# phylo42/RAPPAS

Hardware: AMD Instinct MI355X
Metric: reads placed/sec (whole node), 150 bp DNA vs 10^7-kmer DB (higher is better)
Workload: dtype f32; 1 GPU; C2: DNA k=10, 999 branches, phylo-kmer DB of 786432 keys / 9995042 entries (seed 42), replicated per GPU; 10000000 x 150 symbol reads per GPU per step (uniform, seed 1+rank), keep_at_most=7; reads_per_gpu=10000000

## Files before the change

### rappas_amd/csrc/rk_kernels.hip

```cpp
#include "rk_device.h"
#include "rk_slots24.h"
#include "rk_compact32.h"
#include "rk_translate.h"
#include "rk_masses.h"
#include "rk_samples.h"

#include <type_traits>
#ifndef RK_ROW_NT
#define RK_ROW_NT 0
#endif
#ifndef RK_ROW_AUX
#define RK_ROW_AUX 0
#endif
#ifndef RK_HEADS_MAX_K
#define RK_HEADS_MAX_K 16
#endif
#ifndef RK_ABLATE
#define RK_ABLATE 0
#endif
#include "../../include/rappas_place.h"

namespace rk {

#ifdef RK_STAMPS
__device__ unsigned long long rk_stamp_buf[2 * 4096 * 16];
__device__ __forceinline__ unsigned long long rk_now() {
    unsigned long long t;
    __builtin_amdgcn_sched_barrier(0);
    asm volatile("s_memtime %0\n\ts_waitcnt lgkmcnt(0)" : "=s"(t)::"memory");
    __builtin_amdgcn_sched_barrier(0);
    return t;
}
struct Stamps {
    unsigned long long st_[16] = {0, 0, 0, 0, 0, 0, 0, 0, 0, 0, 0, 0, 0, 0, 0, 0};
    unsigned long long t_ = rk_now();
    __device__ __forceinline__ void mark(int slot) {
        const unsigned long long n_ = rk_now();
        st_[slot] += n_ - t_;
        t_ = n_;
    }
    __device__ __forceinline__ void add(int slot, unsigned long long n) { st_[slot] += n; }
    __device__ __forceinline__ void store(unsigned long long index) const {
        for (int i = 0; i < 16; i++) rk_stamp_buf[index * 16 + i] = st_[i];
    }
};
#else
struct Stamps {
    __device__ __forceinline__ void mark(int) {}
    __device__ __forceinline__ void add(int, unsigned long long) {}
    __device__ __forceinline__ void store(unsigned long long) const {}
};
#endif

__device__ __forceinline__ u32 ord_f32(float f) {
    u32 u = __float_as_uint(f);
    return (u & 0x80000000u) ? ~u : (u | 0x80000000u);
}
__device__ __forceinline__ float unord_f32(u32 o) {
    u32 u = (o & 0x80000000u) ? (o & 0x7FFFFFFFu) : ~o;
    return __uint_as_float(u);
}
__device__ __forceinline__ u64 make_key(u32 raw_score_bits, u32 branch) {
    return ((u64)ord_f32(__uint_as_float(raw_score_bits)) << 32) | (u64)(0xFFFFu - branch);
}
__device__ __forceinline__ u64 shfl64(u64 v, int src, int width) {
    u32 lo = (u32)v, hi = (u32)(v >> 32);
    lo = __shfl(lo, src, width);
    hi = __shfl(hi, src, width);
    return ((u64)hi << 32) | lo;
}
__device__ __forceinline__ u64 shfl_xor64(u64 v, int m, int width) {
    u32 lo = (u32)v, hi = (u32)(v >> 32);
    lo = __shfl_xor(lo, m, width);
    hi = __shfl_xor(hi, m, width);
    return ((u64)hi << 32) | lo;
}
__device__ __forceinline__ double shfl_f64(double v, int src, int width) {
    return __longlong_as_double((long long)shfl64((u64)__double_as_longlong(v), src, width));
}
__device__ __forceinline__ bool tile_order_given(const PlaceArgs &a) { return a.perm != nullptr && *a.keep_order == 0u; }
__device__ __forceinline__ u32 batch_class(const PlaceArgs &a) { return a.keep_order[0] == 0u ? 2u : (a.keep_order[3] != 0u ? 1u : 0u); }
__device__ __forceinline__ bool batch_is_mine(const PlaceArgs &a) {
    if (!a.only_if || !a.perm) return true;
    return ((a.only_if >> batch_class(a)) & 1u) != 0u;
}
__device__ __forceinline__ bool takes_only_marked(const PlaceArgs &a) {
    if (!a.only_marked) return false;
    if (!a.marked_if || !a.perm) return true;
    return ((a.marked_if >> batch_class(a)) & 1u) != 0u;
}
__device__ __forceinline__ u64 tile_read(const PlaceArgs &a, u64 slot, bool given) { return given ? (u64)a.perm[slot] : slot; }
struct ReadHead {
    u32 R, flags, Q;
    float QT;
    bool is_amb, rejected;
};
template <int BITS>
__device__ __forceinline__ void clamp_len(u32 &R, u32 words_per_read) {
    const u32 cap_syms = (words_per_read * 32u) / BITS;
    R = R < cap_syms ? R : cap_syms;
}
template <int BITS>
__device__ __forceinline__ ReadHead read_head(const PlaceArgs &a, u32 R_raw, u32 fin, bool have) {
    const u32 k = a.db.k;
    ReadHead h;
    h.R = R_raw;
    clamp_len<BITS>(h.R, a.words_per_read);
    h.flags = fin & (RK_FLAG_BAD_CHAR | RK_FLAG_AMBIGUOUS | RK_FLAG_TOO_LONG);
    h.is_amb = (fin & RK_FLAG_AMBIGUOUS) != 0;
    h.rejected = (fin & (RK_FLAG_BAD_CHAR | RK_FLAG_TOO_LONG)) != 0;
    if (h.R < k) h.flags |= RK_FLAG_TOO_SHORT;
    h.Q = (have && !h.is_amb && !h.rejected && h.R >= k) ? (h.R - k + 1) : 0u;
    h.QT = (float)(int)h.Q * a.db.T;
    return h;
}
__device__ __forceinline__ bool deferred(const PlaceArgs &a, const ReadHead &h) { return h.is_amb && a.has_ascii && !h.rejected; }
__device__ __forceinline__ void wave_lds_fence() {
    __builtin_amdgcn_fence(__ATOMIC_ACQ_REL, "wavefront");
    __builtin_amdgcn_wave_barrier();
}

template <int G>
__device__ __forceinline__ u64 group_bits(u64 bal, u32 gi) {
    if (G == 64) return bal;
    u32 lo = (u32)bal, hi = (u32)(bal >> 32);
    asm("" : "+v"(lo), "+v"(hi));
    if (G == 32) return gi ? hi : lo;
    constexpr u32 PER = 32 / (G < 32 ? G : 32);
    const u32 half = gi >= PER ? hi : lo;
    return (half >> ((gi % PER) * (u32)G)) & ((1u << (G < 32 ? G : 31)) - 1u);
}
template <int G>
__device__ __forceinline__ int count_below(u64 m, u32 li) {
    if (G <= 32) return __builtin_popcount((u32)m & ((1u << li) - 1u));
    return (int)__builtin_amdgcn_mbcnt_hi((u32)(m >> 32), __builtin_amdgcn_mbcnt_lo((u32)m, 0u));
}
__device__ __forceinline__ u64 bits_below(u32 n) {
    u32 lo = n >= 32u ? 0xFFFFFFFFu : ((1u << (n & 31u)) - 1u);
    u32 hi = n <= 32u ? 0u : (n >= 64u ? 0xFFFFFFFFu : ((1u << ((n - 32u) & 31u)) - 1u));
    asm("" : "+v"(lo), "+v"(hi));
    return ((u64)hi << 32) | lo;
}
__device__ __forceinline__ u64 place_bits(u32 v, u32 sh) {
    u32 lo = sh < 32u ? v << (sh & 31u) : 0u;
    u32 hi = sh >= 32u ? v << ((sh - 32u) & 31u) : ((sh & 31u) ? v >> ((32u - sh) & 31u) : 0u);
    asm("" : "+v"(lo), "+v"(hi));
    return ((u64)hi << 32) | lo;
}
__device__ __forceinline__ bool lane_bit(u64 m, u32 lane) {
    u32 lo = (u32)m, hi = (u32)(m >> 32);
    asm("" : "+v"(lo), "+v"(hi));
    return (((lane & 32u) ? hi : lo) >> (lane & 31u)) & 1u;
}
__device__ __forceinline__ u64 funnel96(u32 w0, u32 w1, u32 w2, u32 sh) {
    return ((u64)__builtin_amdgcn_alignbit(w2, w1, sh) << 32) | __builtin_amdgcn_alignbit(w1, w0, sh);
}

__device__ __forceinline__ void load_entry(const DbView &db, u64 desc, u32 e, u32 &br, float &sc) {
    const unsigned char *base = db.rows + ((desc >> DESC_LEN_BITS) << 3);
    if (db.soa) {
        const u32 len = (u32)desc & DESC_LEN_MASK;
        br = ((const unsigned short *)base)[e];
        sc = ((const float *)(base + 2 * (size_t)len))[e];
    } else {
        const Entry en = ((const Entry *)base)[e];
        br = en.branch ? (en.branch >> 2) - 1u : 0xFFFFu;
        sc = en.score;
    }
}

template <int BITS>
__device__ __forceinline__ u64 extract_code(const u32 *rec, u32 words, u32 j, u32 k) {
    const u32 bit = j * BITS;
    const u32 wi = bit >> 5, sh = bit & 31;
    const u32 last = words - 1;
    const u32 w0 = rec[wi];
    const u32 i1 = wi + 1 < words ? wi + 1 : last;
    u32 w1 = rec[i1];
    w1 = wi + 1 < words ? w1 : 0u;
    const u32 nbits = k * BITS;
    u32 w2 = 0u;
    if (BITS == 5 || nbits + 31 > 64) {
        const u32 i2 = wi + 2 < words ? wi + 2 : last;
        w2 = rec[i2];
        w2 = (wi + 2 < words && nbits + sh > 64) ? w2 : 0u;
    }
    const u64 code = funnel96(w0, w1, w2, sh);
    return nbits >= 64 ? code : (code & ((1ull << nbits) - 1));
}

template <int BITS>
__device__ __forceinline__ u64 dense_index(u64 code, u32 k) {
    if (BITS == 2) return code;
    if (k <= 7) {
        const u32 lo = (u32)code;
        u32 idx = (u32)(code >> 30) & 31u;
        idx = idx * 20u + ((lo >> 25) & 31u);
        idx = idx * 20u + ((lo >> 20) & 31u);
        idx = idx * 20u + ((lo >> 15) & 31u);
        idx = idx * 20u + ((lo >> 10) & 31u);
        idx = idx * 20u + ((lo >> 5) & 31u);
        idx = idx * 20u + (lo & 31u);
// ... 176 lines not shown
            const u32 xw = b - s_lo;
            return (xw < s_win) ? (xw + 1u) * 4u : 0u;
        }
        const u32 t = b - wlo4p4;
        return win ? ((t < w4) ? t + 4u : 0u) : b;
    };
    while (true) {
#pragma unroll
        for (int u = 0; u < U; u++) {
            apply_slot(S, slot_of(br[u]), sc[u], QT, T);
            cursor_issue<G, WIDE, SOA>(c, list, cnt, li, (int)li, rows, br[u], sc[u], s_lo, s_win);
        }
        if (!__any(c.h < cnt)) break;
    }
#pragma unroll
    for (int u = 0; u < U; u++) apply_slot(S, slot_of(br[u]), sc[u], QT, T);
}

template <bool WIDE> struct ItemT { typedef u32 type; };
template <> struct ItemT<true> { typedef u64 type; };

template <int G, bool WIDE>
__device__ __forceinline__ typename ItemT<WIDE>::type make_item(u64 off8, u32 n) {
    if (WIDE) return (typename ItemT<WIDE>::type)((off8 << DESC_LEN_BITS) | n);
    return (typename ItemT<WIDE>::type)((u32)(off8 >> 3) << 4 | (n >> 3));
}

template <int G, bool WIDE>
__device__ __forceinline__ void chunk_issue(typename ItemT<WIDE>::type it, bool in, u32 li, u32 li8,
                                            const unsigned char *rows, u32 &br, float &sc) {
    typedef typename OffsetT<WIDE>::type off_t;
    bool ok;
    off_t eo;
    if (WIDE) {
        const u32 n = (u32)it & DESC_LEN_MASK;
        ok = in && li < n;
        eo = (off_t)(((u64)it >> DESC_LEN_BITS) << 3) + li8;
    } else {
        ok = in && (li >> 3) < ((u32)it & 15u);
        eo = (off_t)((((u32)it & ~15u) << 2) + li8);
    }
    eo = ok ? eo : (off_t)0;
    if (RK_ABLATE & 16) eo = 0;
    const uint2 e = *(const uint2 *)(rows + eo);
    br = e.x;
    sc = __uint_as_float(e.y);
}

template <int G, int U, bool WIDE>
__device__ __forceinline__ void accumulate_chunks(u32 *S, u32 nb, const typename ItemT<WIDE>::type *items, int cnt,
                                                  u32 li, const unsigned char *rows, float QT, float T) {
    typedef typename ItemT<WIDE>::type item_t;
    const u32 li8 = li * 8;
    u32 br[U];
    float sc[U];
    item_t it[U];
#pragma unroll
    for (int u = 0; u < U; u++) chunk_issue<G, WIDE>(items[u], u < cnt, li, li8, rows, br[u], sc[u]);
#pragma unroll
    for (int u = 0; u < U; u++) it[u] = items[U + u];
    int s0 = 0;
    while (true) {
#pragma unroll
        for (int u = 0; u < U; u++) {
            apply_slot(S, br[u], sc[u], QT, T);
            chunk_issue<G, WIDE>(it[u], s0 + U + u < cnt, li, li8, rows, br[u], sc[u]);
            it[u] = items[s0 + 2 * U + u];
        }
        s0 += U;
        if (!__any(s0 < cnt)) break;
    }
}

constexpr u32 ITEM_FILLER = 0xFFFFFF00u;
typedef u32 v2u32 __attribute__((ext_vector_type(2)));

__device__ __forceinline__ __amdgpu_buffer_rsrc_t rows_resource(const DbView &db) {
    return __builtin_amdgcn_make_buffer_rsrc((void *)db.rows, (short)0, (int)(u32)db.rows_bytes, 0x00020000);
}

template <int G, int U, bool MONO, bool WIN = false, bool D24 = false>
__device__ __forceinline__ void accumulate_units(u32 *S, const u32 *items, int wcnt, u32 li,
                                                 __amdgpu_buffer_rsrc_t rs, float QT, float T, u32 wlo4p4 = 4u, u32 w4 = 0xFFFFFFFFu) {
    static_assert(!D24 || (G == 16 && !WIN), "dense units: 16-lane groups, whole trees");
    static_assert(rk_slots24::SLOT_BITS == SLOT24_BITS, "rk_slots24.h unpacks the slot words rk_device.h defines");
    const u32 li8 = li * 8;
    const u32 my_unit = li >> 4;
    const rk_slots24::Shifts sh24 = rk_slots24::lane_shifts(li);
    u32 sb[U], it[U];
    float sc[U];
    auto issue = [&](u32 item, u32 &b, float &v) {
        u32 off = item + li8;
        if (G > 16) off = (my_unit <= (item & 7u)) ? (item & ~127u) + li8 : ITEM_FILLER;
        if (RK_ABLATE & 16) off = li8;
        const v2u32 e = __builtin_amdgcn_raw_buffer_load_b64(rs, (int)off, 0, RK_ROW_AUX);
        b = e.x;
        v = __uint_as_float(e.y);
    };
    auto slot_of = [&](u32 b) {
        if (!WIN) return b;
        const u32 t = b - wlo4p4;
        return (t < w4) ? t + 4u : 0u;
    };
    auto prepare = [&](float v, u32 *&pa, u32 *&pb) {
        const int w = (int)__float_as_uint(v);
        const u32 r = (u32)__builtin_amdgcn_update_dpp(w, w, 0x128, 0xF, 0x3, false);
        const rk_slots24::Slots s = rk_slots24::lane_slots(sh24, r);
        pa = S + s.a;
        pb = S + s.b;
    };
#pragma unroll
    for (int u = 0; u < U; u++) issue(items[u], sb[u], sc[u]);
#pragma unroll
    for (int u = 0; u < U; u++) it[u] = items[U + u];
    int s0 = 0;
    if (D24) {
        u32 *pa, *pb;
        prepare(sc[0], pa, pb);
        while (true) {
#pragma unroll
            for (int u = 0; u < U; u++) {
                u32 *na, *nb;
                if (RK_ABLATE & 8) {
                    asm volatile("" ::"v"(pa), "v"(pb), "v"(sb[u]), "v"(sc[u]));
                    prepare(sc[(u + 1) % U], na, nb);
                } else {
                    const u32 oa = *pa, ob = *pb;
                    prepare(sc[(u + 1) % U], na, nb);
                    *pa = __float_as_uint(touch_base<MONO>(oa, QT) + __uint_as_float(sb[u]));
                    *pb = __float_as_uint(touch_base<MONO>(ob, QT) + sc[u]);
                }
                issue(it[u], sb[u], sc[u]);
                it[u] = items[s0 + 2 * U + u];
                pa = na;
                pb = nb;
            }
            s0 += U;
            if (s0 >= wcnt) break;
        }
        return;
    }
    while (true) {
#pragma unroll
        for (int u = 0; u < U; u++) {
            apply_slot<MONO>(S, slot_of(sb[u]), sc[u], QT, T);
            issue(it[u], sb[u], sc[u]);
            it[u] = items[s0 + 2 * U + u];
        }
        s0 += U;
        if (s0 >= wcnt) break;
    }
}

template <int S>
__device__ __forceinline__ u32 row_ror32(u32 v) {
    return (u32)__builtin_amdgcn_update_dpp(0, (int)v, 0x120 + S, 0xF, 0xF, false);
}
template <int G, int S>
__device__ __forceinline__ u64 group_rotate(u64 v, u32 li) {
    if (G == 16) {
        return ((u64)row_ror32<S>((u32)(v >> 32)) << 32) | row_ror32<S>((u32)v);
    } else {
        return shfl64(v, (int)((li + G - S) % G), G);
    }
}
template <int G, int S>
struct RankAbove {
    static __device__ __forceinline__ int run(u64 v, u32 li) {
        return ((group_rotate<G, S>(v, li) > v) ? 1 : 0) + RankAbove<G, S - 1>::run(v, li);
    }
};
template <int G>
struct RankAbove<G, 0> {
    static __device__ __forceinline__ int run(u64, u32) { return 0; }
};
template <int G>
__device__ __forceinline__ u64 group_max(u64 v) {
    if (G == 16) {
        u64 o;
        o = ((u64)row_ror32<8>((u32)(v >> 32)) << 32) | row_ror32<8>((u32)v); v = o > v ? o : v;
        o = ((u64)row_ror32<4>((u32)(v >> 32)) << 32) | row_ror32<4>((u32)v); v = o > v ? o : v;
        o = ((u64)row_ror32<2>((u32)(v >> 32)) << 32) | row_ror32<2>((u32)v); v = o > v ? o : v;
        o = ((u64)row_ror32<1>((u32)(v >> 32)) << 32) | row_ror32<1>((u32)v); v = o > v ? o : v;
        return v;
    } else {
#pragma unroll
        for (int s = 1; s < G; s <<= 1) {
            u64 o = shfl_xor64(v, s, G);
            v = o > v ? o : v;
        }
        return v;
    }
}

template <int G>
__device__ __forceinline__ int rank_candidates(const u64 *list, int c, u64 *win, int K, u32 li) {
    if (c <= G) {
        const u64 mine = ((int)li < c) ? list[li] : 0ull;
        const int rank = RankAbove<G, G - 1>::run(mine, li);
        if (mine != 0 && rank < K) win[rank] = mine;
    } else {
        for (int j = (int)li; j < c; j += G) {
            const u64 mine = list[j];
            int rank = 0;
            for (int t = 0; t < c; t++) rank += (list[t] > mine) ? 1 : 0;
            if (rank < K) win[rank] = mine;
        }
    }
    wave_lds_fence();
    return c < K ? c : K;
}

template <int G>
__device__ __forceinline__ int select_topk_scan(u32 *S, u32 ns, u32 li, u32 gi, int K, u64 *list, int cap, u64 &win_key, Stamps &stamps) {
    const u32 nb = ns;
    u64 *win = list + (cap - 16);
    const int capc = cap - 16;
    const uint4 *S4 = (const uint4 *)S;
    uint4 *S4w = (uint4 *)S;
    const u32 n4 = (nb + 3) / 4;
    float mo = -INFINITY;
    u32 mi = 0xFFFFFFFFu;
    for (u32 q = li; q < n4; q += G) {
        const uint4 v4 = S4[q];
        const u32 i = 4 * q;
        const float v[4] = {__uint_as_float(v4.x), __uint_as_float(v4.y), __uint_as_float(v4.z), __uint_as_float(v4.w)};
#pragma unroll
        for (int e = 0; e < 4; e++) {
            const bool gt = (v[e] > mo) && (i + e < nb);
            mo = gt ? v[e] : mo;
            mi = gt ? i + e : mi;
        }
    }
    const u64 km = (mi != 0xFFFFFFFFu) ? make_key(__float_as_uint(mo), mi - 1u) : 0ull;
    const int rank = RankAbove<G, G - 1>::run(km, li);
    u64 tau = group_max<G>((rank == K - 1) ? km : 0ull);
    int c = 0;
    const uint4 reset4 = make_uint4(S_UNTOUCHED, S_UNTOUCHED, S_UNTOUCHED, S_UNTOUCHED);
    for (u32 q0 = 0; q0 < n4; q0 += G) {
        const u32 q = q0 + li;
        uint4 v4 = reset4;
        if (q < n4) { v4 = S4[q]; S4w[q] = reset4; }
        const u32 i = 4 * q;
        const u32 raw[4] = {v4.x, v4.y, v4.z, v4.w};
        u64 key[4];
        bool any = false;
#pragma unroll
        for (int e = 0; e < 4; e++) {
            key[e] = (raw[e] != S_UNTOUCHED && i + e < nb) ? make_key(raw[e], i + e - 1u) : 0ull;
            any = any || (key[e] != 0 && key[e] >= tau);
        }
        if (group_bits<G>(__ballot(any), gi) == 0) continue;
#pragma unroll
        for (int e = 0; e < 4; e++) {
            const bool cand = key[e] != 0 && key[e] >= tau;
            const u64 sub = group_bits<G>(__ballot(cand), gi);
            if (sub == 0) continue;
            if (c + G > capc) {
                wave_lds_fence();
                const int kept = rank_candidates<G>(list, c, win, K, li);
                if ((int)li < kept) list[li] = win[li];
                if (kept == K) tau = win[K - 1];
                wave_lds_fence();
                c = kept;
            }
            const bool still = cand && key[e] >= tau;
            const u64 sub2 = group_bits<G>(__ballot(still), gi);
            if (still) list[c + count_below<G>(sub2, li)] = key[e];
            c += __builtin_popcountll(sub2);
        }
    }
    wave_lds_fence();
    const int num = rank_candidates<G>(list, c, win, K, li);
    win_key = ((int)li < num) ? win[li] : 0ull;
    wave_lds_fence();
    return num;
}

__device__ __forceinline__ u64 mask_eq0(u32 v) {
    u64 m;
    asm("v_cmp_eq_u32_e64 %0, 0, %1" : "=s"(m) : "v"(v));
    return m;
}
__device__ __forceinline__ u64 mask_eq_lo16(u32 a, u32 b) {
    u64 m;
    asm("v_cmp_eq_u16_e64 %0, %1, %2" : "=s"(m) : "v"(a), "v"(b));
    return m;
}
__device__ __forceinline__ u64 mask_ge(u32 a, u32 b) {
    u64 m;
    asm("v_cmp_ge_u32_e64 %0, %1, %2" : "=s"(m) : "v"(a), "s"(b));
    return m;
}
__device__ __forceinline__ u32 mask_select(u32 if_clear, u32 if_set, u64 m) {
    u32 r;
    asm("v_cndmask_b32_e64 %0, %1, %2, %3" : "=v"(r) : "v"(if_clear), "v"(if_set), "s"(m));
    return r;
}
__device__ __forceinline__ u32 lds_cas_issue(u32 at, u32 expect, u32 put) {
    u32 r;
    asm volatile("ds_cmpst_rtn_b32 %0, %1, %2, %3" : "=v"(r) : "v"(at), "v"(expect), "v"(put) : "memory");
    return r;
}
template <int N>
__device__ __forceinline__ void lds_cas_wait(u32 (&r)[N]) {
    asm volatile("s_waitcnt lgkmcnt(0)" : : : "memory");
// ... 675 lines not shown
        if (BITS * 12 + 31 > 64) {
            w2 = __shfl(recw, (int)((wi + 2) & 15u), 16);
            w2 = (wi + 2 < 16 && nbits + sh > 64) ? w2 : 0u;
        }
        const u64 c = funnel96(w0, w1, w2, sh);
        code[u] = nbits >= 64 ? c : (c & ((1ull << nbits) - 1));
    }
}

template <int BITS, int PU>
__device__ __forceinline__ void record_indices(u32 recw, u32 pos, u32 li, u32 k, u32 Q, u32 (&idx)[PU]) {
    if (BITS == 2) {
        const u32 mask = (k >= 16) ? 0xFFFFFFFFu : ((1u << (2 * k)) - 1u);
        if (PU <= 15 && pos == 0) {
            u32 w[PU + 1];
            Batch0Words<PU, 0>::run(recw, w);
#pragma unroll
            for (int u = 0; u < PU; u++) idx[u] = __builtin_amdgcn_alignbit(w[u + 1], w[u], 2 * li) & mask;
            return;
        }
#pragma unroll
        for (int u = 0; u < PU; u++) {
            const u32 j0 = pos + u * 16 + li;
            const u32 j = j0 < Q ? j0 : 0u;
            const u32 wi = j >> 4, sh = (j & 15u) * 2u;
            const u32 w0 = __shfl(recw, (int)(wi & 15u), 16);
            u32 w1 = __shfl(recw, (int)((wi + 1) & 15u), 16);
            w1 = wi + 1 < 16 ? w1 : 0u;
            idx[u] = __builtin_amdgcn_alignbit(w1, w0, sh) & mask;
        }
        return;
    }
    u64 code[PU];
    record_codes<BITS, PU>(recw, pos, li, k, Q, code);
#pragma unroll
    for (int u = 0; u < PU; u++) idx[u] = (u32)dense_index<BITS>(code[u], k);
}

template <int PU, bool C32>
struct ProbeBatch {
    RawSlot raw[PU];
    u32 j[C32 ? PU : 1];
    u64 code[C32 ? 1 : PU];
};
template <int PU, bool C32>
struct RowBatch {
    u32 unit[C32 ? PU : 1], n[C32 ? PU : 1];
    u64 desc[C32 ? 1 : PU];
};
__device__ __forceinline__ u64 unit_desc(u32 unit, u32 n) { return n ? ((u64)(unit * ROW_UNIT) << DESC_LEN_BITS) | (u64)(n * ROW_UNIT) : 0ull; }

template <int BITS, int TM, int U, int PU, bool D24 = false>
__global__ void __launch_bounds__(256) place_packed16_kernel(PlaceArgs a) {
    constexpr int G = 16, NG = 4;
    static_assert(TM != TM_HASH, "direct tables only");
    static_assert(!D24 || TM == TM_COMPACT, "the dense view carries a compact table");
    if (!batch_is_mine(a)) return;
    extern __shared__ u32 lds[];
    const bool perm_given = tile_order_given(a);
    const u32 lane = threadIdx.x & 63;
    const u32 wave = threadIdx.x >> 6;
    const u32 waves_per_block = blockDim.x >> 6;
    const u32 gi = lane / G, li = lane % G;
    const u32 wave_words = NG * (a.s_stride + 2 * a.list_cap);
    u32 *wbase = lds + wave * wave_words;
    u32 *S = wbase + gi * a.s_stride;
    u64 *list = (u64 *)(wbase + NG * a.s_stride) + gi * a.list_cap;
    u32 *items = (u32 *)list;
    const u32 nb = a.db.n_branches;
    const u32 k = a.db.k;
    const float T = a.db.T;
    const __amdgpu_buffer_rsrc_t rows_rs = rows_resource(a.db);
    const int cap_items = (int)(a.list_cap * 2) - 3 * U - 2;
    const int cap_rows = (int)a.list_cap - 1;
    const u32 wpr = a.words_per_read;

    for (u32 i = li; i < a.s_stride; i += G) S[i] = S_UNTOUCHED;
    wave_lds_fence();

    const u64 n_tiles = (a.n_reads + NG - 1) / NG;
    const u64 wave_global = (u64)blockIdx.x * waves_per_block + wave;
    const u64 wave_count = (u64)gridDim.x * waves_per_block;

    auto load_tile = [&](u64 tile, u32 &recw, u32 &R, u32 &fin, bool &have) {
        const u64 slot = tile * NG + gi;
        have = tile < n_tiles && slot < a.n_reads;
        const u64 r = have ? tile_read(a, slot, perm_given) : 0ull;
        recw = 0; R = 0; fin = 0;
        if (have) {
            if (li < wpr) recw = a.packed[r * wpr + li];
            R = a.lens ? a.lens[r] : a.fixed_len;
            fin = a.flags_in ? a.flags_in[r] : 0u;
        }
    };
    constexpr bool C32 = TM == TM_COMPACT;
    const bool nib = a.db.compact_nib != 0;
    auto fetch_batch = [&](u32 recw, u32 pos, u32 Q, ProbeBatch<PU, C32> &pb) {
        if constexpr (C32) {
            u32 idx[PU];
            record_indices<BITS, PU>(recw, pos, li, k, Q, idx);
            const unsigned char *table = (const unsigned char *)a.db.compact;
#pragma unroll
            for (int u = 0; u < PU; u++) {
                const rk_compact32::Pos p = nib ? rk_compact32::locate_nib(idx[u]) : rk_compact32::locate_byte(idx[u]);
                pb.j[u] = p.j;
                pb.raw[u].v = *(const uint4 *)(table + p.blk * 16u);
            }
        } else {
            record_codes<BITS, PU>(recw, pos, li, k, Q, pb.code);
#pragma unroll
            for (int u = 0; u < PU; u++) pb.raw[u] = lookup_fetch<BITS, TM>(a.db, pb.code[u]);
        }
    };
    auto decode_batch = [&](const ProbeBatch<PU, C32> &pb, u32 pos, u32 Q, RowBatch<PU, C32> &rows) {
        if constexpr (C32) {
#pragma unroll
            for (int u = 0; u < PU; u++) {
                const uint4 v = pb.raw[u].v;
                const rk_compact32::Row r = nib ? rk_compact32::decode_nib(v.x, v.y, v.z, v.w, pb.j[u]) : rk_compact32::decode_byte(v.x, v.y, v.z, v.w, pb.j[u]);
                rows.unit[u] = r.unit;
                rows.n[u] = r.n;
            }
        } else {
#pragma unroll
            for (int u = 0; u < PU; u++) {
                const u32 j = pos + u * G + li;
                const u64 d = lookup_decode<BITS, TM>(a.db, pb.raw[u], pb.code[u]);
                rows.desc[u] = j < Q ? d : 0ull;
            }
        }
    };

    Stamps stamps;
    u32 c_recw, c_R, c_fin;
    bool c_have;
    RowBatch<PU, C32> rows0;
    {
        load_tile(wave_global, c_recw, c_R, c_fin, c_have);
        ProbeBatch<PU, C32> pb;
        const u32 Q0 = read_head<BITS>(a, c_R, c_fin, c_have).Q;
        fetch_batch(c_recw, 0u, Q0, pb);
        decode_batch(pb, 0u, Q0, rows0);
    }

    for (u64 tile = wave_global; tile < n_tiles; tile += wave_count) {
        const bool have = c_have;
        const u64 r = have ? tile_read(a, tile * NG + gi, perm_given) : 0ull;
        const u32 fin = c_fin;
        const ReadHead h = read_head<BITS>(a, c_R, fin, have);
        const u32 Q = h.Q;
        const float QT = h.QT;

        int cnt = 0;
        auto flush = [&]() {
            int wcnt = __builtin_amdgcn_readlane(cnt, 0);
            wcnt = max(wcnt, __builtin_amdgcn_readlane(cnt, 32));
            wcnt = max(wcnt, __builtin_amdgcn_readlane(cnt, 16));
            wcnt = max(wcnt, __builtin_amdgcn_readlane(cnt, 48));
            for (int i = cnt + (int)li; i < wcnt + 2 * U; i += G) items[i] = ITEM_FILLER;
            wave_lds_fence();
            if (a.db.mono) accumulate_units<G, U, true, false, D24>(S, items, wcnt, li, rows_rs, QT, T);
            else accumulate_units<G, U, false, false, D24>(S, items, wcnt, li, rows_rs, QT, T);
            wave_lds_fence();
            cnt = 0;
        };
        auto emit_batch = [&](const RowBatch<PU, C32> &rows, u32 pos, bool more) {
            u32 nch[PU], excl[PU], rb[PU];
            int total = 0;
            bool wide_rows = false;
#pragma unroll
            for (int u = 0; u < PU; u++) {
                if constexpr (C32) nch[u] = pos + u * G + li < Q ? rows.n[u] : 0u;
                else nch[u] = (((u32)rows.desc[u] & DESC_LEN_MASK) + G - 1) >> 4;
                if constexpr (C32) rb[u] = rows.unit[u] * 128u;
                else rb[u] = (u32)(rows.desc[u] >> DESC_LEN_BITS) * 8u;
                if (!(C32 && nib)) wide_rows = wide_rows || nch[u] > 15u;
            }
            auto row_scan = [](u32 v) {
                v += (u32)__builtin_amdgcn_update_dpp(0, (int)v, 0x111, 0xF, 0xF, true);
                v += (u32)__builtin_amdgcn_update_dpp(0, (int)v, 0x112, 0xF, 0xF, true);
                v += (u32)__builtin_amdgcn_update_dpp(0, (int)v, 0x114, 0xF, 0xF, true);
                v += (u32)__builtin_amdgcn_update_dpp(0, (int)v, 0x118, 0xF, 0xF, true);
                return v;
            };
            if (!__any(wide_rows)) {
#pragma unroll
                for (int u0 = 0; u0 < PU; u0 += 4) {
                    u32 packed = nch[u0];
                    if (u0 + 1 < PU) packed |= nch[u0 + 1 < PU ? u0 + 1 : u0] << 8;
                    if (u0 + 2 < PU) packed |= nch[u0 + 2 < PU ? u0 + 2 : u0] << 16;
                    if (u0 + 3 < PU) packed |= nch[u0 + 3 < PU ? u0 + 3 : u0] << 24;
                    const u32 incl = row_scan(packed);
                    const u32 tot = row_bcast32<15>(incl);
#pragma unroll
                    for (int b = 0; b < 4; b++) {
                        if (u0 + b < PU) {
                            const int u = u0 + b < PU ? u0 + b : u0;
                            excl[u] = (u32)total + ((incl >> (8 * b)) & 0xFFu) - nch[u];
                            total += (int)((tot >> (8 * b)) & 0xFFu);
                        }
                    }
                }
            } else {
#pragma unroll
                for (int u = 0; u < PU; u++) {
                    const u32 incl = row_scan(nch[u]);
                    excl[u] = (u32)total + incl - nch[u];
                    total += (int)row_bcast32<15>(incl);
                }
            }
            if (__any(more && cnt + total > cap_items)) flush();
            if (D24 && __any(more && total > cap_items)) {
                for (u32 done = 0; __any(done < (u32)total);) {
                    const u32 room = (u32)(cap_items - cnt);
#pragma unroll
                    for (int u = 0; u < PU; u++) {
                        for (u32 c = 0; __any(c < nch[u]); c++) {
                            const u32 x = excl[u] + c - done;
                            if (c < nch[u] && x < room) items[cnt + (int)x] = rb[u] + c * 128u;
                        }
                    }
                    const u32 take = min((u32)total - done, room);
                    cnt += (int)take;
                    done += take;
                    if (__any(done < (u32)total)) flush();
                }
            } else if (__any(more && total > cap_items)) {
                const int per_part = cap_rows / G;
                for (int u_lo = 0; u_lo < PU; u_lo += per_part) {
                    int rc = 0;
#pragma unroll
                    for (int u = 0; u < PU; u++) {
                        const bool part = u >= u_lo && u < u_lo + per_part;
                        const bool hit = part && nch[u] != 0;
                        const u64 bal = __ballot(hit);
                        const u64 sub = group_bits<G>(bal, gi);
                        u64 d;
                        if constexpr (C32) d = unit_desc(rows.unit[u], nch[u]);
                        else d = rows.desc[u];
                        if (hit) list[rc + count_below<G>(sub, li)] = d;
                        rc += __builtin_popcountll(sub);
                    }
                    if (li == 0) list[rc] = 0;
                    wave_lds_fence();
                    if (__any(rc > 0)) accumulate_list<G, U, false>(S, nb, list, rc, li, a.db.rows, QT, T);
                    wave_lds_fence();
                }
            } else {
#pragma unroll
                for (int u = 0; u < PU; u++) {
                    const int base = cnt + (int)excl[u];
                    if (nch[u] > 0) items[base] = rb[u];
                    if (nch[u] > 1) items[base + 1] = rb[u] + 128u;
                    for (u32 c = 2; __any(c < nch[u]); c++)
                        if (c < nch[u]) items[base + (int)c] = rb[u] + c * 128u;
                }
                cnt += total;
            }
        };

        stamps.mark(0);
        emit_batch(rows0, 0u, Q > 0);
        for (u32 pos = PU * G; __any(pos < Q); pos += PU * G) {
            ProbeBatch<PU, C32> pb;
            RowBatch<PU, C32> rows;
            fetch_batch(c_recw, pos, Q, pb);
            __builtin_amdgcn_sched_barrier(0);
            decode_batch(pb, pos, Q, rows);
            emit_batch(rows, pos, pos < Q);
        }
        stamps.mark(2);
        load_tile(tile + wave_count, c_recw, c_R, c_fin, c_have);
        if (__any(cnt > 0)) flush();
        stamps.mark(4);
        ProbeBatch<PU, C32> npb;
        const u32 nQ = read_head<BITS>(a, c_R, c_fin, c_have).Q;
        fetch_batch(c_recw, 0u, nQ, npb);
        __builtin_amdgcn_sched_barrier(0);
        stamps.mark(1);

        u64 win_key;
        int numBest = 0;
        if (RK_ABLATE & 2) { win_key = list[0]; for (u32 i = li; i <= nb; i += G) S[i] = S_UNTOUCHED; }
        else numBest = select_topk<G>(S, nb, li, gi, (int)a.keep_at_most, list, (int)a.list_cap, win_key, stamps);
        wave_lds_fence();
        stamps.mark(5);
        decode_batch(npb, 0u, nQ, rows0);
        if constexpr (C32) {
#pragma unroll
            for (int u = 0; u < PU; u++) asm volatile("" : "+v"(rows0.unit[u]), "+v"(rows0.n[u]));
        }
        __builtin_amdgcn_sched_barrier(0);
        stamps.mark(3);
        if (have && !deferred(a, h)) weigh_and_store<G>(a, r, li, numBest, win_key, h.flags);
        stamps.mark(6);
    }
    if (lane == 0 && wave_global < 4096) stamps.store(wave_global);
}

constexpr int RETILE_BINS = 64;
template <int BITS>
__device__ __forceinline__ u32 retile_read_key(const PlaceArgs &a, u64 r, u32 &spread, u32 *with_row = nullptr) {
    const u32 k = a.db.k, wpr = a.words_per_read;
    const ReadHead h = read_head<BITS>(a, a.lens ? a.lens[r] : a.fixed_len, a.flags_in ? a.flags_in[r] : 0u, true);
    u32 key = 0;
    spread = 0;
    if (h.flags == 0u) {
        const u32 Q = h.Q;
        const u32 *rec = a.packed + r * wpr;
        constexpr int NS = 7;
        u32 w[NS];
#pragma unroll
        for (int i = 0; i < NS; i++) {
            const u32 p_ = (u32)(((u64)(Q - 1) * (u32)i) / (NS - 1));
            w[i] = a.db.winspec[(u32)dense_index<BITS>(extract_code<BITS>(rec, wpr, p_, k), k)] & 63u;
        }
        u32 best = 0, best_n = 0;
#pragma unroll
        for (int i = 0; i < NS; i++) {
            u32 n_ = 0;
#pragma unroll
            for (int j = 0; j < NS; j++) n_ += (w[j] != 0u && (w[i] > w[j] ? w[i] - w[j] : w[j] - w[i]) <= 1u) ? 1u : 0u;
            n_ = w[i] != 0u ? n_ : 0u;
            best = n_ > best_n ? w[i] : best;
            best_n = max(best_n, n_);
        }
        key = best;
        if (with_row) {
            u32 nz = 0;
#pragma unroll
            for (int i = 0; i < NS; i++) nz += w[i] != 0u ? 1u : 0u;
            *with_row = nz;
        }
        spread = best_n < 3u ? 1u : 0u;
    }
    return key;
}
template <int BITS>
__global__ void __launch_bounds__(256) retile_sample_kernel(PlaceArgs a, u32 *hist) {
    const u64 r = ((u64)blockIdx.x * blockDim.x + threadIdx.x) * 64u;
    u32 spread = 0, with_row = 0;
    const bool on = r < a.n_reads;
    if (on) (void)retile_read_key<BITS>(a, r, spread, &with_row);
    const u64 sp = __ballot(on && spread != 0u), al = __ballot(on);
    for (int o = 32; o > 0; o >>= 1) with_row += (u32)__shfl_down((int)with_row, o, 64);
    if ((threadIdx.x & 63u) == 0) {
        if (sp) atomicAdd(&hist[RETILE_BINS], (u32)__builtin_popcountll(sp));
        if (al) atomicAdd(&hist[RETILE_BINS + 2], (u32)__builtin_popcountll(al));
        if (with_row) atomicAdd(&hist[RETILE_BINS + 3], with_row);
    }
}
__global__ void retile_decide_kernel(u32 *hist, u32 sparse_q16) {
    if (threadIdx.x == 0) {
        hist[RETILE_BINS + 1] = (hist[RETILE_BINS] * 2u > hist[RETILE_BINS + 2]) ? 1u : 0u;
        hist[RETILE_BINS + 4] = ((u64)hist[RETILE_BINS + 3] * 65536ull <= (u64)hist[RETILE_BINS + 2] * 7ull * (u64)sparse_q16) ? 1u : 0u;
    }
}
template <int BITS>
__global__ void __launch_bounds__(256) retile_key_kernel(PlaceArgs a, unsigned char *keys, u32 *hist) {
    if (hist[RETILE_BINS + 1]) return;
    __shared__ u32 h[RETILE_BINS];
    if (threadIdx.x < RETILE_BINS) h[threadIdx.x] = 0;
    __syncthreads();
    for (u64 r = (u64)blockIdx.x * blockDim.x + threadIdx.x; r < a.n_reads; r += (u64)gridDim.x * blockDim.x) {
        u32 spread;
        const u32 key = retile_read_key<BITS>(a, r, spread);
        keys[r] = (unsigned char)key;
        atomicAdd(&h[key], 1u);
    }
    __syncthreads();
    if (threadIdx.x < RETILE_BINS && h[threadIdx.x]) atomicAdd(&hist[threadIdx.x], h[threadIdx.x]);
}
__global__ void __launch_bounds__(64) retile_scan_kernel(u32 *hist, u32 *cursor) {
    const u32 t = threadIdx.x;
    u32 v = hist[t], incl = v;
    for (int s = 1; s < 64; s <<= 1) {
        const u32 o = (u32)__shfl_up((int)incl, s, 64);
        if ((int)t >= s) incl += o;
    }
    cursor[t] = incl - v;
}
__global__ void __launch_bounds__(256) retile_scatter_kernel(u64 n_reads, const unsigned char *keys, const u32 *hist, u32 *cursor, u32 *perm) {
    __shared__ u32 cnt[RETILE_BINS], base[RETILE_BINS];
    if (hist[RETILE_BINS + 1]) return;
    for (u64 r0 = (u64)blockIdx.x * blockDim.x; r0 < n_reads; r0 += (u64)gridDim.x * blockDim.x) {
        const u64 r = r0 + threadIdx.x;
        if (threadIdx.x < RETILE_BINS) cnt[threadIdx.x] = 0;
        __syncthreads();
        u32 key = 0, rank = 0;
        if (r < n_reads) {
            key = keys[r];
            rank = atomicAdd(&cnt[key], 1u);
        }
        __syncthreads();
        if (threadIdx.x < RETILE_BINS && cnt[threadIdx.x]) base[threadIdx.x] = atomicAdd(&cursor[threadIdx.x], cnt[threadIdx.x]);
        __syncthreads();
        if (r < n_reads) perm[base[key] + rank] = (u32)r;
        __syncthreads();
    }
}

__global__ void __launch_bounds__(256) compact_marks_kernel(const unsigned char *marks, u64 n_tiles, u32 *list, u32 *ctl) {
    const u32 lane = threadIdx.x & 63;
    const u64 stride = (u64)gridDim.x * blockDim.x;
    const u64 rounds = (n_tiles + stride - 1) / stride;
    for (u64 it = 0; it < rounds; it++) {
        const u64 t = it * stride + (u64)blockIdx.x * blockDim.x + threadIdx.x;
        const bool m = t < n_tiles && marks[t] != 0;
        const u64 bal = __ballot(m);
// ... 2073 lines not shown
```

Baseline: 417.6 million reads/s.

## Issue first unit loads early during emit and use tiled tail accumulation

Adds a UnitRing-based accumulation path (units_issue/units_run) that separates issuing the first U row loads from consuming them. In the dense-24 path, once the first four probe batches' item offsets are known, it writes those items and issues the initial buffer loads early, so their latency overlaps the remaining scan and item writing. The flush path skips re-issuing loads when the ring is already live. It also adds a TILE tail that processes leftover items in pairs instead of full U-wide blocks, which cuts wasted filler loads at the cost of more code paths and register pressure.

```diff
diff --git a/rappas_amd/csrc/rk_kernels.hip b/rappas_amd/csrc/rk_kernels.hip
--- a/rappas_amd/csrc/rk_kernels.hip
+++ b/rappas_amd/csrc/rk_kernels.hip
@@ -40,6 +40,7 @@
         t_ = n_;
     }
     __device__ __forceinline__ void add(int slot, unsigned long long n) { st_[slot] += n; }
+    __device__ __forceinline__ Stamps *ptr() { return this; }
     __device__ __forceinline__ void store(unsigned long long index) const {
         for (int i = 0; i < 16; i++) rk_stamp_buf[index * 16 + i] = st_[i];
     }
@@ -48,6 +49,7 @@
 struct Stamps {
     __device__ __forceinline__ void mark(int) {}
     __device__ __forceinline__ void add(int, unsigned long long) {}
+    __device__ __forceinline__ Stamps *ptr() { return nullptr; }
     __device__ __forceinline__ void store(unsigned long long) const {}
 };
 #endif
@@ -530,6 +532,109 @@
     }
 }
 
+template <int U>
+struct UnitRing {
+    u32 sb[U], it[U];
+    float sc[U];
+};
+template <int G>
+__device__ __forceinline__ void unit_issue(__amdgpu_buffer_rsrc_t rs, u32 item, u32 li, u32 &b, float &v) {
+    const u32 li8 = li * 8;
+    u32 off = item + li8;
+    if (G > 16) off = ((li >> 4) <= (item & 7u)) ? (item & ~127u) + li8 : ITEM_FILLER;
+    if (RK_ABLATE & 16) off = li8;
+    const v2u32 e = __builtin_amdgcn_raw_buffer_load_b64(rs, (int)off, 0, RK_ROW_AUX);
+    b = e.x;
+    v = __uint_as_float(e.y);
+}
+template <int G, int U>
+__device__ __forceinline__ void units_issue(UnitRing<U> &r, const u32 *items, u32 li, __amdgpu_buffer_rsrc_t rs) {
+#pragma unroll
+    for (int u = 0; u < U; u++) unit_issue<G>(rs, items[u], li, r.sb[u], r.sc[u]);
+#pragma unroll
+    for (int u = 0; u < U; u++) r.it[u] = items[U + u];
+}
+template <int F, int N, bool B> struct StepBlock { static constexpr int first = F, steps = N; static constexpr bool feed = B; };
+template <int G, int U, bool MONO, bool WIN = false, bool D24 = false, bool TILE = false>
+__device__ __forceinline__ void units_run(UnitRing<U> &r, u32 *S, const u32 *items, int wcnt, u32 li, __amdgpu_buffer_rsrc_t rs, float QT, float T,
+                                          u32 wlo4p4 = 4u, u32 w4 = 0xFFFFFFFFu, Stamps *stamps = nullptr) {
+    static_assert(!D24 || (G == 16 && !WIN), "dense units: 16-lane groups, whole trees");
+    static_assert(!TILE || U == 8, "a tail of up to three pairs of steps");
+    static_assert(rk_slots24::SLOT_BITS == SLOT24_BITS, "rk_slots24.h unpacks the slot words rk_device.h defines");
+    const rk_slots24::Shifts sh24 = rk_slots24::lane_shifts(li);
+    u32(&sb)[U] = r.sb;
+    u32(&it)[U] = r.it;
+    float(&sc)[U] = r.sc;
+    auto issue = [&](u32 item, u32 &b, float &v) { unit_issue<G>(rs, item, li, b, v); };
+    auto slot_of = [&](u32 b) {
+        if (!WIN) return b;
+        const u32 t = b - wlo4p4;
+        return (t < w4) ? t + 4u : 0u;
+    };
+    auto prepare = [&](float v, u32 *&pa, u32 *&pb) {
+        const int w = (int)__float_as_uint(v);
+        const u32 r = (u32)__builtin_amdgcn_update_dpp(w, w, 0x128, 0xF, 0x3, false);
+        const rk_slots24::Slots s = rk_slots24::lane_slots(sh24, r);
+        pa = S + s.a;
+        pb = S + s.b;
+    };
+    if (stamps) {
+        asm volatile("" ::"v"(sc[0]));
+        stamps->mark(7);
+    }
+    int s0 = 0;
+    u32 *pa = S, *pb = S;
+    if (D24) prepare(sc[0], pa, pb);
+    auto block = [&](auto kind) __attribute__((always_inline)) {
+        constexpr int F = decltype(kind)::first, N = decltype(kind)::steps;
+        constexpr bool FEED = decltype(kind)::feed;
+#pragma unroll
+        for (int u = F; u < F + N; u++) {
+            if (D24) {
+                u32 *na = pa, *nb = pb;
+                if (RK_ABLATE & 8) {
+                    asm volatile("" ::"v"(pa), "v"(pb), "v"(sb[u]), "v"(sc[u]));
+                    prepare(sc[(u + 1) % U], na, nb);
+                } else {
+                    const u32 oa = *pa, ob = *pb;
+                    prepare(sc[(u + 1) % U], na, nb);
+                    *pa = __float_as_uint(touch_base<MONO>(oa, QT) + __uint_as_float(sb[u]));
+                    *pb = __float_as_uint(touch_base<MONO>(ob, QT) + sc[u]);
+                }
+                pa = na;
+                pb = nb;
+            } else {
+                apply_slot<MONO>(S, slot_of(sb[u]), sc[u], QT, T);
+            }
+            if (FEED) {
+                issue(it[u], sb[u], sc[u]);
+                it[u] = items[s0 + 2 * U + u];
+            }
+        }
+    };
+    if (TILE) {
+        while (wcnt - s0 > U - 2) {
+            block(StepBlock<0, U, true>());
+            s0 += U;
+        }
+        const int left = wcnt - s0;
+        if (left > 0) {
+            block(StepBlock<0, 2, false>());
+            if (left > 2) {
+                block(StepBlock<2, 2, false>());
+                if (left > 4) block(StepBlock<4, 2, false>());
+            }
+        }
+        if (stamps) stamps->add(12, (unsigned long long)(s0 + (left > 0 ? (left + 1) & ~1 : 0)));
+        return;
+    }
+    while (true) {
+        block(StepBlock<0, U, true>());
+        s0 += U;
+        if (s0 >= wcnt) break;
+    }
+    if (stamps) stamps->add(12, (unsigned long long)s0);
+}
 template <int S>
 __device__ __forceinline__ u32 row_ror32(u32 v) {
     return (u32)__builtin_amdgcn_update_dpp(0, (int)v, 0x120 + S, 0xF, 0xF, false);
@@ -1511,22 +1616,32 @@
         const float QT = h.QT;
 
         int cnt = 0;
-        auto flush = [&]() {
+        UnitRing<U> ring;
+        bool ring_live = false;
+        constexpr bool EARLY = D24;
+        auto flush = [&]() __attribute__((always_inline)) {
             int wcnt = __builtin_amdgcn_readlane(cnt, 0);
             wcnt = max(wcnt, __builtin_amdgcn_readlane(cnt, 32));
             wcnt = max(wcnt, __builtin_amdgcn_readlane(cnt, 16));
             wcnt = max(wcnt, __builtin_amdgcn_readlane(cnt, 48));
             for (int i = cnt + (int)li; i < wcnt + 2 * U; i += G) items[i] = ITEM_FILLER;
             wave_lds_fence();
-            if (a.db.mono) accumulate_units<G, U, true, false, D24>(S, items, wcnt, li, rows_rs, QT, T);
-            else accumulate_units<G, U, false, false, D24>(S, items, wcnt, li, rows_rs, QT, T);
+            stamps.mark(10);
+            if (!ring_live) units_issue<G, U>(ring, items, li, rows_rs);
+            ring_live = false;
+            stamps.mark(11);
+            if (a.db.mono) units_run<G, U, true, false, D24, true>(ring, S, items, wcnt, li, rows_rs, QT, T, 4u, 0xFFFFFFFFu, stamps.ptr());
+            else units_run<G, U, false, false, D24, true>(ring, S, items, wcnt, li, rows_rs, QT, T, 4u, 0xFFFFFFFFu, stamps.ptr());
+            stamps.mark(4);
             wave_lds_fence();
+            stamps.mark(10);
             cnt = 0;
         };
         auto emit_batch = [&](const RowBatch<PU, C32> &rows, u32 pos, bool more) {
             u32 nch[PU], excl[PU], rb[PU];
             int total = 0;
             bool wide_rows = false;
+            bool early = false;
 #pragma unroll
             for (int u = 0; u < PU; u++) {
                 if constexpr (C32) nch[u] = pos + u * G + li < Q ? rows.n[u] : 0u;
@@ -1542,6 +1657,16 @@
                 v += (u32)__builtin_amdgcn_update_dpp(0, (int)v, 0x118, 0xF, 0xF, true);
                 return v;
             };
+            auto write_rows = [&](int u_lo, int u_hi) {
+#pragma unroll
+                for (int u = u_lo; u < u_hi; u++) {
+                    const int base = cnt + (int)excl[u];
+                    if (nch[u] > 0) items[base] = rb[u];
+                    if (nch[u] > 1) items[base + 1] = rb[u] + 128u;
+                    for (u32 c = 2; __any(c < nch[u]); c++)
+                        if (c < nch[u]) items[base + (int)c] = rb[u] + c * 128u;
+                }
+            };
             if (!__any(wide_rows)) {
 #pragma unroll
                 for (int u0 = 0; u0 < PU; u0 += 4) {
@@ -1559,6 +1684,15 @@
                             total += (int)((tot >> (8 * b)) & 0xFFu);
                         }
                     }
+                    if constexpr (EARLY) {
+                        if (u0 == 0 && PU > 4 && pos == 0 && !__any(total < 2 * U || total > cap_items)) {
+                            write_rows(0, 4);
+                            wave_lds_fence();
+                            units_issue<G, U>(ring, items, li, rows_rs);
+                            __builtin_amdgcn_sched_barrier(0);
+                            ring_live = early = true;
+                        }
+                    }
                 }
             } else {
 #pragma unroll
@@ -1568,7 +1702,7 @@
                     total += (int)row_bcast32<15>(incl);
                 }
             }
-            if (__any(more && cnt + total > cap_items)) flush();
+            if (!early && __any(more && cnt + total > cap_items)) flush();
             if (D24 && __any(more && total > cap_items)) {
                 for (u32 done = 0; __any(done < (u32)total);) {
                     const u32 room = (u32)(cap_items - cnt);
@@ -1606,14 +1740,8 @@
                     wave_lds_fence();
                 }
             } else {
-#pragma unroll
-                for (int u = 0; u < PU; u++) {
-                    const int base = cnt + (int)excl[u];
-                    if (nch[u] > 0) items[base] = rb[u];
-                    if (nch[u] > 1) items[base + 1] = rb[u] + 128u;
-                    for (u32 c = 2; __any(c < nch[u]); c++)
-                        if (c < nch[u]) items[base + (int)c] = rb[u] + c * 128u;
-                }
+                if (!early) write_rows(0, PU < 4 ? PU : 4);
+                write_rows(PU < 4 ? PU : 4, PU);
                 cnt += total;
             }
         };
```

Result: faster. 425.2 million reads/s (median of 6 runs) (+1.8%).
